# RohanVKashyap/resolution-pde

Measured on AMD Instinct MI355X. Metric: training samples/sec, FFNO2D NS 256^2, higher is better.
Workload: dtype f32; 1 GPU; FFNO2D(1,1,width=64,n_layers=4,n_modes=20,factor=4,ff_weight_norm,n_ff_layers=3,layer_norm,dropout=0.1) train step on [B,1,256,256] Gaussian random fields (BASELINE configs[2]); batch_per_gpu=32, global_batch=32, optimizer=AdamW lr=1e-3 (rpde.optim.FlatAdamW: torch.optim.AdamW's rule, one kernel), parallelism=single, grad_bucket_bytes=6828576, target=input advanced by a fixed spectral filter (utils/synthetic.py:advance)

## Files before the change

resolution-pde_amd/csrc/wgrad_h2.hip:

```cpp
#include "h2.h"
#include "pointwise.h"
#include "wgrad_h2.h"

namespace rpde {

constexpr int WG_WAVES = 8;
constexpr int WG_PANEL = 8192;
constexpr int WG_BLOCKS = 256;

struct WgP {
  const float* a;
  const float* b;
  float* slabs;
  long npts;
  long steps;
  int M, N, nchunk;
  const float* w;
  float* gx;
  int early;
};

template <int PA, int PB, int WM, int WN, int TM, int TN, bool ACT, bool DG = false>
__global__ __launch_bounds__(64 * WG_WAVES, 2) void k_wgrad_h2(const WgP P) {
  static_assert(!DG || (PB == 1 && PA * 2 <= 8), "data gradient: N = 64, M <= 256");
  constexpr int WFRAG = DG ? PA * 2 * 4 * 2048 : 0;
  static_assert(WM * WN == WG_WAVES && PA + PB <= WG_WAVES, "eight waves, one panel per loader wave");
  static_assert(WM * TM * 16 == PA * 64 && WN * TN * 16 == PB * 64, "wave tiles cover the block");
  static_assert((TM * 16) % 64 == 0 || 64 % (TM * 16) == 0, "a wave tile stays inside one panel or covers whole panels");
  constexpr int STAGE = (PA + PB) * WG_PANEL;
  __shared__ __attribute__((aligned(16))) char smem[2 * STAGE + WFRAG];
  __shared__ int einfo[2][WG_WAVES];
  __shared__ float wmax[WG_WAVES];
  const int tid = threadIdx.x, l = tid & 63, wave = tid >> 6, g = l >> 4, li = l & 15;
  const int chunk = blockIdx.x, mblock = blockIdx.y;
  const long s0 = P.steps * chunk / P.nchunk, s1 = P.steps * (chunk + 1) / P.nchunk;

  const bool loader = wave < PA + PB, isA = wave < PA;
  const int ld = isA ? P.M : P.N;
  const float* __restrict__ src = isA ? P.a + mblock * (64 * PA) + 64 * wave : P.b + 64 * (wave - PA);
  src += (long)g * ld + 4 * li;
  float4 buf[8];
  int e_run = 15;
  auto issue = [&](long s) {
    if (!loader || s >= s1) return;
    const float* __restrict__ q0 = src + s * 32 * ld;
    if ((s + 1) * 32 <= P.npts) {
#pragma unroll
      for (int i = 0; i < 8; ++i) buf[i] = *reinterpret_cast<const float4*>(q0 + (long)(4 * i) * ld);
    } else {
#pragma unroll
      for (int i = 0; i < 8; ++i)
        buf[i] = s * 32 + 4 * i + g < P.npts ? *reinterpret_cast<const float4*>(q0 + (long)(4 * i) * ld) : make_float4(0.f, 0.f, 0.f, 0.f);
    }
  };
  auto convert = [&](int st) {
    if (!loader) return;
    if (ACT && !isA) {
#pragma unroll
      for (int i = 0; i < 8; ++i) { buf[i].x = gelu_f(buf[i].x); buf[i].y = gelu_f(buf[i].y); buf[i].z = gelu_f(buf[i].z); buf[i].w = gelu_f(buf[i].w); }
    }
    float m = 0.f;
#pragma unroll
    for (int i = 0; i < 8; ++i) m = fmaxf(fmaxf(m, fmaxf(fabsf(buf[i].x), fabsf(buf[i].y))), fmaxf(fabsf(buf[i].z), fabsf(buf[i].w)));
    m = wave_max(m);
    e_run = max(e_run, (int)(__float_as_uint(m) >> 23) & 0xff);
    e_run = min(e_run, 254);
    const float scale = __uint_as_float((unsigned)(268 - e_run) << 23);
    char* const dst = smem + st * STAGE + wave * WG_PANEL;
#pragma unroll
    for (int i = 0; i < 8; ++i) {
      uint2 hi, lo;
      h2_split4(buf[i].x * scale, buf[i].y * scale, buf[i].z * scale, buf[i].w * scale, hi, lo);
      const int off = stage_off(4 * i + g, li);
      *reinterpret_cast<uint2*>(dst + off) = hi;
      *reinterpret_cast<uint2*>(dst + 4096 + off) = lo;
    }
    if (l == 0) einfo[st][wave] = e_run;
  };

  const int wm = wave / WN, wn = wave % WN;
  const int m_off = wm * TM * 16, n_off = wn * TN * 16;
  const int pa = m_off >> 6, ta0 = (m_off & 63) >> 4, pb = PA + (n_off >> 6), tb0 = (n_off & 63) >> 4;
  const int q = li >> 2, pp = li & 3;
  const int tsw = ((q >> 1) & 1) | ((g & 1) << 1);
  const int trow = (8 * g + q) * 128 + pp * 8;
  typedef s16x4v __attribute__((address_space(3))) * lds_tr;
  auto frag = [&](const char* panel, int tile, f16x8& hi, f16x8& lo) {
    const char* t = panel + trow + ((tile ^ tsw) << 5);
    union { struct { s16x4v a, b; } h; f16x8 v; } uh, ul;
    uh.h.a = __builtin_amdgcn_ds_read_tr16_b64_v4i16((lds_tr)(t));
    uh.h.b = __builtin_amdgcn_ds_read_tr16_b64_v4i16((lds_tr)(t + 512));
    ul.h.a = __builtin_amdgcn_ds_read_tr16_b64_v4i16((lds_tr)(t + 4096));
    ul.h.b = __builtin_amdgcn_ds_read_tr16_b64_v4i16((lds_tr)(t + 4096 + 512));
    hi = uh.v; lo = ul.v;
  };
  f32x4v acc[TM][TN];
#pragma unroll
  for (int i = 0; i < TM; ++i)
#pragma unroll
    for (int j = 0; j < TN; ++j) acc[i][j] = (f32x4v){0.f, 0.f, 0.f, 0.f};
  constexpr int NPA = (TM * 16 + 63) / 64;
  static_assert(TN * 16 <= 64, "one B panel per wave tile");
  int ea_used[NPA], eb_used = 15;
#pragma unroll
  for (int k = 0; k < NPA; ++k) ea_used[k] = 15;

  char* const wfrag = smem + 2 * STAGE;
  float w_inv = 1.f;
  if (DG && s0 < s1) {
    constexpr int NF = PA * 2 * 4 * 64 / (64 * WG_WAVES);
    float wv[NF][8];
    float m = 0.f;
#pragma unroll
    for (int r = 0; r < NF; ++r) {
      const int c = tid + r * 64 * WG_WAVES, fl = c & 63, nt = (c >> 6) & 3, ks = c >> 8;
#pragma unroll
      for (int j = 0; j < 8; ++j) {
        wv[r][j] = P.w[(long)(32 * ks + 8 * (fl >> 4) + j) * P.N + 16 * nt + (fl & 15)];
        m = fmaxf(m, fabsf(wv[r][j]));
      }
    }
    m = wave_max(m);
    if (l == 0) wmax[wave] = m;
    __syncthreads();
    m = 0.f;
#pragma unroll
    for (int i = 0; i < WG_WAVES; ++i) m = fmaxf(m, wmax[i]);
    float w_scale;
    h2_scale(m, 0, w_scale, w_inv);
#pragma unroll
    for (int r = 0; r < NF; ++r) {
      const int c = tid + r * 64 * WG_WAVES, fl = c & 63, nt = (c >> 6) & 3, ks = c >> 8;
      uint2 h0, l0, h1, l1;
      h2_split4(wv[r][0] * w_scale, wv[r][1] * w_scale, wv[r][2] * w_scale, wv[r][3] * w_scale, h0, l0);
      h2_split4(wv[r][4] * w_scale, wv[r][5] * w_scale, wv[r][6] * w_scale, wv[r][7] * w_scale, h1, l1);
      char* d = wfrag + (ks * 4 + nt) * 2048 + fl * 16;
      *reinterpret_cast<uint4*>(d) = make_uint4(h0.x, h0.y, h1.x, h1.y);
      *reinterpret_cast<uint4*>(d + 1024) = make_uint4(l0.x, l0.y, l1.x, l1.y);
    }
  }
  const int dg_mt = wave & 1, dg_nt = wave >> 1;

  const bool early_convert = (P.early >> __builtin_amdgcn_readfirstlane(wave)) & 1;
  if (s0 < s1) {
    issue(s0);
    convert(0);
    issue(s0 + 1);
    lds_barrier();
    for (long s = s0; s < s1; ++s) {
      const int cur = (int)(s - s0) & 1;
      const char* const stage = smem + cur * STAGE;
      if (early_convert && s + 1 < s1) {
        convert(cur ^ 1);
        issue(s + 2);
      }
      const int eb = __builtin_amdgcn_readfirstlane(einfo[cur][pb]);
#pragma unroll
      for (int k = 0; k < NPA; ++k) {
        const int ea = __builtin_amdgcn_readfirstlane(einfo[cur][pa + k]);
        if (ea + eb != ea_used[k] + eb_used) {
          const int d = (ea_used[k] + eb_used) - (ea + eb);
          const float f = d > -126 ? __uint_as_float((unsigned)(127 + d) << 23) : 0.f;
#pragma unroll
          for (int i = 0; i < TM; ++i)
            if (((ta0 + i) >> 2) == k) {
#pragma unroll
              for (int j = 0; j < TN; ++j) acc[i][j] *= f;
            }
        }
        ea_used[k] = ea;
      }
      eb_used = eb;
      f16x8 bh[TN], bl[TN];
#pragma unroll
      for (int j = 0; j < TN; ++j) frag(stage + (pb + ((tb0 + j) >> 2)) * WG_PANEL, (tb0 + j) & 3, bh[j], bl[j]);
#pragma unroll
      for (int i = 0; i < TM; ++i) {
        f16x8 ah, al;
        frag(stage + (pa + ((ta0 + i) >> 2)) * WG_PANEL, (ta0 + i) & 3, ah, al);
#pragma unroll
        for (int j = 0; j < TN; ++j) acc[i][j] = h2_mfma32(ah, al, bh[j], bl[j], acc[i][j]);
      }
      if (DG) {
        f32x4v tot = (f32x4v){0.f, 0.f, 0.f, 0.f};
        const int row = 16 * dg_mt + li;
#pragma unroll
        for (int k = 0; k < PA; ++k) {
          f32x4v part = (f32x4v){0.f, 0.f, 0.f, 0.f};
#pragma unroll
          for (int h = 0; h < 2; ++h) {
            const char* pa_ = stage + k * WG_PANEL + stage_off(row, 2 * (4 * h + g));
            const f16x8 ah = *reinterpret_cast<const f16x8*>(pa_), al = *reinterpret_cast<const f16x8*>(pa_ + 4096);
            const char* wb = wfrag + ((2 * k + h) * 4 + dg_nt) * 2048 + l * 16;
            const f16x8 bh = *reinterpret_cast<const f16x8*>(wb), bl = *reinterpret_cast<const f16x8*>(wb + 1024);
            part = h2_mfma32(ah, al, bh, bl, part);
          }
          const int ek = __builtin_amdgcn_readfirstlane(einfo[cur][k]);
          const float fk = __uint_as_float((unsigned)(ek - 14) << 23) * w_inv;
          tot += part * fk;
        }
        float t0 = tot[0], t1 = tot[1], t2 = tot[2], t3 = tot[3];
        quad_transpose(t0, t1, t2, t3);
        const long pq = s * 32 + 16 * dg_mt + 4 * g + (li & 3);
        if (pq < P.npts) *reinterpret_cast<float4*>(P.gx + pq * P.N + 16 * dg_nt + 4 * (li >> 2)) = make_float4(t0, t1, t2, t3);
      }
      if (!early_convert && s + 1 < s1) {
        convert(cur ^ 1);
        issue(s + 2);
      }
      lds_barrier();
    }
  }

  const float fb = __uint_as_float((unsigned)(eb_used - 14) << 23);
  float* __restrict__ out = P.slabs + (long)chunk * P.M * P.N + (long)(mblock * (64 * PA) + m_off) * P.N + n_off;
#pragma unroll
  for (int i = 0; i < TM; ++i) {
    const float fa = __uint_as_float((unsigned)(ea_used[(ta0 + i) >> 2] - 14) << 23);
#pragma unroll
    for (int j = 0; j < TN; ++j)
#pragma unroll
      for (int r = 0; r < 4; ++r) out[(long)(16 * i + 4 * g + r) * P.N + 16 * j + li] = acc[i][j][r] * fa * fb;
  }
}

bool wgrad_h2_ok(long P, int out_f, int in_f) {
  if (switch_off("RPDE_WGRAD_H2") || P < 32L * WG_BLOCKS) return false;
  return (out_f == 256 && in_f == 256) || (out_f == 256 && in_f == 64) || (out_f == 64 && in_f == 256);
}

static int wg_chunks(int, int) { return WG_BLOCKS; }

static int wg_early_mask(int out_f, int in_f) {
  return out_f == 256 && in_f == 256 ? 0xF0 : (out_f == 64 ? 0x0E : 0x00);
}

size_t wgrad_h2_slab_floats(long P, int out_f, int in_f) {
  return wgrad_h2_ok(P, out_f, in_f) ? (size_t)wg_chunks(out_f, in_f) * out_f * in_f : 0;
}

template <int PA, int PB, int WM, int WN, int TM, int TN>
static void wg_launch(const WgP& p, int mblocks, bool act, hipStream_t st) {
  const dim3 grid(p.nchunk, mblocks);
  if (act) hipLaunchKernelGGL((k_wgrad_h2<PA, PB, WM, WN, TM, TN, true>), grid, dim3(64 * WG_WAVES), 0, st, p);
  else hipLaunchKernelGGL((k_wgrad_h2<PA, PB, WM, WN, TM, TN, false>), grid, dim3(64 * WG_WAVES), 0, st, p);
}

bool wgrad_h2_dgrad_ok(long P, int out_f, int in_f) { return wgrad_h2_ok(P, out_f, in_f) && out_f == 256 && in_f == 64; }

int wgrad_h2_dgrad(const float* gy, const float* h, const float* w, float* gw, float* gx, long P, int in_f, int out_f,
                   float* slabs, hipStream_t st, FoldJobs* defer) {
  RPDE_CHECK_ARG(wgrad_h2_dgrad_ok(P, out_f, in_f) && slabs && w && gx, "wgrad_h2_dgrad: unsupported shape");
  WgP p;
  p.a = gy; p.b = h; p.slabs = slabs; p.npts = P; p.steps = (P + 31) / 32; p.M = out_f; p.N = in_f; p.nchunk = WG_BLOCKS;
  p.early = wg_early_mask(out_f, in_f);
  p.w = w; p.gx = gx;
  hipLaunchKernelGGL((k_wgrad_h2<4, 1, 4, 2, 4, 2, false, true>), dim3(p.nchunk, 1), dim3(64 * WG_WAVES), 0, st, p);
  RPDE_LAUNCH_CHECK();
  if (defer && defer->add(slabs, gw, out_f * in_f, p.nchunk, (long)out_f * in_f)) return RPDE_OK;
  return reduce_slabs(slabs, gw, (long)out_f * in_f, p.nchunk, (long)out_f * in_f, 1.f, 0, st);
}

int wgrad_h2(const float* gy, const float* h, float* gw, long P, int in_f, int out_f, int act_b, float* slabs, hipStream_t st,
             FoldJobs* defer) {
  RPDE_CHECK_ARG(wgrad_h2_ok(P, out_f, in_f) && slabs, "wgrad_h2: unsupported shape");
  RPDE_CHECK_ARG(act_b == RPDE_ACT_IDENTITY || act_b == RPDE_ACT_GELU, "wgrad_h2: activation %d", act_b);
  WgP p;
  p.a = gy; p.b = h; p.slabs = slabs; p.npts = P; p.steps = (P + 31) / 32; p.M = out_f; p.N = in_f; p.nchunk = wg_chunks(out_f, in_f);
  p.early = wg_early_mask(out_f, in_f);
  p.w = nullptr; p.gx = nullptr;
  const bool act = act_b == RPDE_ACT_GELU;
  if (out_f == 256 && in_f == 256) wg_launch<4, 4, 2, 4, 8, 4>(p, 1, act, st);
  else if (out_f == 256) wg_launch<4, 1, 4, 2, 4, 2>(p, 1, act, st);
  else wg_launch<1, 4, 1, 8, 4, 2>(p, 1, act, st);
  RPDE_LAUNCH_CHECK();
  if (defer && defer->add(slabs, gw, out_f * in_f, p.nchunk, (long)out_f * in_f)) return RPDE_OK;
  return reduce_slabs(slabs, gw, (long)out_f * in_f, p.nchunk, (long)out_f * in_f, 1.f, 0, st);
}

}
```

Measured before the change: 1012 samples/s.

## Hold weight fragments in registers and stage data-gradient rows through LDS

In the fused weight-gradient plus data-gradient kernel, the W fragments now stay in registers instead of being read from LDS on every step. Each step's gx tile is written to a double-buffered, XOR-swizzled LDS buffer, and the non-loader waves flush it to global memory one step later as full contiguous rows. The early-convert wave mask for this path also changes. The aim is to cut LDS traffic and scattered global stores on the critical path, at the cost of extra registers per wave. A timestamp profiling mode is added but compiled only under RPDE_STAMPS.

After: 1018 samples/s (median of 6 runs). Within noise of the previous version (+0.6%).

```diff
diff --git a/profiles/wg_stamps.py b/profiles/wg_stamps.py
--- /dev/null
+++ b/profiles/wg_stamps.py
@@ -0,0 +1,31 @@
+#!/usr/bin/env python3
+import ctypes as C
+import os
+import sys
+
+REPO = os.path.dirname(os.path.dirname(os.path.abspath(__file__)))
+for p in (REPO, os.path.join(REPO, "resolution-pde_amd")):
+    sys.path.insert(0, p)
+import numpy as np
+import torch
+from rpde import _lib
+from models.custom_layer import FeedForward
+
+lib = _lib.load()
+ff = FeedForward(64, 4, n_layers=3, layer_norm=True, dropout=0.1).to("cuda")
+x = torch.randn(32, 256, 256, 64, device="cuda").requires_grad_(True)
+res = torch.randn(32, 256, 256, 64, device="cuda")
+g = torch.randn(32, 256, 256, 64, device="cuda")
+for _ in range(3):
+    ff(x, residual=res).backward(g)
+torch.cuda.synchronize()
+buf = (C.c_ulonglong * 64)()
+lib.rpde_debug_wg_stamps.argtypes = [C.c_void_p]
+_lib.check(lib.rpde_debug_wg_stamps(buf), "stamps")
+t = np.array(buf, dtype=np.uint64).reshape(8, 8).astype(np.int64)
+names = ["early convert", "main product", "data gradient", "load wait", "convert", "issue + gx rows", "barrier"]
+print("cycles per step (s_memtime ticks), workgroup 128, steps", int(t[0, 7]))
+print("wave " + " ".join(f"{n:>15s}" for n in names) + "          total")
+for w in range(8):
+    per = t[w, :7] / max(1, t[w, 7])
+    print(f"{w:4d} " + " ".join(f"{v:15.0f}" for v in per) + f" {per.sum():14.0f}")
diff --git a/resolution-pde_amd/csrc/wgrad_h2.hip b/resolution-pde_amd/csrc/wgrad_h2.hip
--- a/resolution-pde_amd/csrc/wgrad_h2.hip
+++ b/resolution-pde_amd/csrc/wgrad_h2.hip
@@ -7,6 +7,14 @@
 constexpr int WG_WAVES = 8;
 constexpr int WG_PANEL = 8192;
 constexpr int WG_BLOCKS = 256;
+
+#ifdef RPDE_STAMPS
+constexpr int WG_NSTAMP = 8;
+__device__ unsigned long long g_wgstamps[WG_WAVES * WG_NSTAMP];
+#define WGSTAMP(i) do { if (DG) { const unsigned long long t_ = __builtin_amdgcn_s_memtime(); st_acc[i] += t_ - st_last; st_last = t_; } } while (0)
+#else
+#define WGSTAMP(i) do {} while (0)
+#endif
 
 struct WgP {
   const float* a;
@@ -23,12 +31,12 @@
 template <int PA, int PB, int WM, int WN, int TM, int TN, bool ACT, bool DG = false>
 __global__ __launch_bounds__(64 * WG_WAVES, 2) void k_wgrad_h2(const WgP P) {
   static_assert(!DG || (PB == 1 && PA * 2 <= 8), "data gradient: N = 64, M <= 256");
-  constexpr int WFRAG = DG ? PA * 2 * 4 * 2048 : 0;
   static_assert(WM * WN == WG_WAVES && PA + PB <= WG_WAVES, "eight waves, one panel per loader wave");
   static_assert(WM * TM * 16 == PA * 64 && WN * TN * 16 == PB * 64, "wave tiles cover the block");
   static_assert((TM * 16) % 64 == 0 || 64 % (TM * 16) == 0, "a wave tile stays inside one panel or covers whole panels");
   constexpr int STAGE = (PA + PB) * WG_PANEL;
-  __shared__ __attribute__((aligned(16))) char smem[2 * STAGE + WFRAG];
+  constexpr int GXBUF = 32 * 64 * 4;
+  __shared__ __attribute__((aligned(16))) char smem[2 * STAGE + (DG ? 2 * GXBUF : 0)];
   __shared__ int einfo[2][WG_WAVES];
   __shared__ float wmax[WG_WAVES];
   const int tid = threadIdx.x, l = tid & 63, wave = tid >> 6, g = l >> 4, li = l & 15;
@@ -105,21 +113,20 @@
 #pragma unroll
   for (int k = 0; k < NPA; ++k) ea_used[k] = 15;
 
-  char* const wfrag = smem + 2 * STAGE;
+  const int dg_mt = wave & 1, dg_nt = wave >> 1;
+  constexpr int NKS = DG ? PA * 2 : 1;
+  f16x8 wh[NKS], wl[NKS];
   float w_inv = 1.f;
   if (DG && s0 < s1) {
-    constexpr int NF = PA * 2 * 4 * 64 / (64 * WG_WAVES);
-    float wv[NF][8];
+    float wv[NKS][8];
     float m = 0.f;
 #pragma unroll
-    for (int r = 0; r < NF; ++r) {
-      const int c = tid + r * 64 * WG_WAVES, fl = c & 63, nt = (c >> 6) & 3, ks = c >> 8;
+    for (int ks = 0; ks < NKS; ++ks)
 #pragma unroll
       for (int j = 0; j < 8; ++j) {
-        wv[r][j] = P.w[(long)(32 * ks + 8 * (fl >> 4) + j) * P.N + 16 * nt + (fl & 15)];
-        m = fmaxf(m, fabsf(wv[r][j]));
-      }
-    }
+        wv[ks][j] = P.w[(long)(32 * ks + 8 * g + j) * P.N + 16 * dg_nt + li];
+        m = fmaxf(m, fabsf(wv[ks][j]));
+      }
     m = wave_max(m);
     if (l == 0) wmax[wave] = m;
     __syncthreads();
@@ -129,17 +136,29 @@
     float w_scale;
     h2_scale(m, 0, w_scale, w_inv);
 #pragma unroll
-    for (int r = 0; r < NF; ++r) {
-      const int c = tid + r * 64 * WG_WAVES, fl = c & 63, nt = (c >> 6) & 3, ks = c >> 8;
-      uint2 h0, l0, h1, l1;
-      h2_split4(wv[r][0] * w_scale, wv[r][1] * w_scale, wv[r][2] * w_scale, wv[r][3] * w_scale, h0, l0);
-      h2_split4(wv[r][4] * w_scale, wv[r][5] * w_scale, wv[r][6] * w_scale, wv[r][7] * w_scale, h1, l1);
-      char* d = wfrag + (ks * 4 + nt) * 2048 + fl * 16;
-      *reinterpret_cast<uint4*>(d) = make_uint4(h0.x, h0.y, h1.x, h1.y);
-      *reinterpret_cast<uint4*>(d + 1024) = make_uint4(l0.x, l0.y, l1.x, l1.y);
+    for (int ks = 0; ks < NKS; ++ks) {
+#pragma unroll
+      for (int j = 0; j < 8; ++j) wv[ks][j] *= w_scale;
+      h2_frag(wv[ks], wh[ks], wl[ks]);
     }
   }
-  const int dg_mt = wave & 1, dg_nt = wave >> 1;
+
+  char* const gxs = smem + 2 * STAGE;
+  auto gx_flush = [&](long sp, int b) {
+    constexpr int W0 = PA + PB, NW = WG_WAVES - W0;
+    static_assert(!DG || NW > 0, "data gradient: at least one wave without a panel");
+    if (!DG || wave < W0) return;
+#pragma unroll
+    for (int rg = 0; rg < 8; rg += NW) {
+      const int r = rg + wave - W0;
+      if (r < 8) {
+        const int prow = 4 * r + g;
+        const float4 v = *reinterpret_cast<const float4*>(gxs + b * GXBUF + prow * 256 + ((li ^ ((prow & 3) << 2)) << 4));
+        const long pq = sp * 32 + prow;
+        if (pq < P.npts) *reinterpret_cast<float4*>(P.gx + pq * P.N + 4 * li) = v;
+      }
+    }
+  };
 
   const bool early_convert = (P.early >> __builtin_amdgcn_readfirstlane(wave)) & 1;
   if (s0 < s1) {
@@ -147,6 +166,9 @@
     convert(0);
     issue(s0 + 1);
     lds_barrier();
+#ifdef RPDE_STAMPS
+    unsigned long long st_acc[WG_NSTAMP] = {0, 0, 0, 0, 0, 0, 0, 0}, st_last = __builtin_amdgcn_s_memtime();
+#endif
     for (long s = s0; s < s1; ++s) {
       const int cur = (int)(s - s0) & 1;
       const char* const stage = smem + cur * STAGE;
@@ -154,6 +176,7 @@
         convert(cur ^ 1);
         issue(s + 2);
       }
+      WGSTAMP(0);
       const int eb = __builtin_amdgcn_readfirstlane(einfo[cur][pb]);
 #pragma unroll
       for (int k = 0; k < NPA; ++k) {
@@ -181,6 +204,7 @@
 #pragma unroll
         for (int j = 0; j < TN; ++j) acc[i][j] = h2_mfma32(ah, al, bh[j], bl[j], acc[i][j]);
       }
+      WGSTAMP(1);
       if (DG) {
         f32x4v tot = (f32x4v){0.f, 0.f, 0.f, 0.f};
         const int row = 16 * dg_mt + li;
@@ -191,9 +215,7 @@
           for (int h = 0; h < 2; ++h) {
             const char* pa_ = stage + k * WG_PANEL + stage_off(row, 2 * (4 * h + g));
             const f16x8 ah = *reinterpret_cast<const f16x8*>(pa_), al = *reinterpret_cast<const f16x8*>(pa_ + 4096);
-            const char* wb = wfrag + ((2 * k + h) * 4 + dg_nt) * 2048 + l * 16;
-            const f16x8 bh = *reinterpret_cast<const f16x8*>(wb), bl = *reinterpret_cast<const f16x8*>(wb + 1024);
-            part = h2_mfma32(ah, al, bh, bl, part);
+            part = h2_mfma32(ah, al, wh[2 * k + h], wl[2 * k + h], part);
           }
           const int ek = __builtin_amdgcn_readfirstlane(einfo[cur][k]);
           const float fk = __uint_as_float((unsigned)(ek - 14) << 23) * w_inv;
@@ -201,15 +223,32 @@
         }
         float t0 = tot[0], t1 = tot[1], t2 = tot[2], t3 = tot[3];
         quad_transpose(t0, t1, t2, t3);
-        const long pq = s * 32 + 16 * dg_mt + 4 * g + (li & 3);
-        if (pq < P.npts) *reinterpret_cast<float4*>(P.gx + pq * P.N + 16 * dg_nt + 4 * (li >> 2)) = make_float4(t0, t1, t2, t3);
-      }
+        const int prow = 16 * dg_mt + 4 * g + (li & 3), c = 4 * dg_nt + (li >> 2);
+        *reinterpret_cast<float4*>(gxs + cur * GXBUF + prow * 256 + ((c ^ ((prow & 3) << 2)) << 4)) = make_float4(t0, t1, t2, t3);
+      }
+      WGSTAMP(2);
+#ifdef RPDE_STAMPS
+      if (DG) asm volatile("s_waitcnt vmcnt(0)" ::: "memory");
+      WGSTAMP(3);
+#endif
       if (!early_convert && s + 1 < s1) {
         convert(cur ^ 1);
+        WGSTAMP(4);
         issue(s + 2);
       }
+      if (DG && s > s0) gx_flush(s - 1, cur ^ 1);
+      WGSTAMP(5);
       lds_barrier();
-    }
+      WGSTAMP(6);
+    }
+#ifdef RPDE_STAMPS
+    if (DG && blockIdx.x == WG_BLOCKS / 2 && l == 0) {
+#pragma unroll
+      for (int i = 0; i < WG_NSTAMP - 1; ++i) g_wgstamps[wave * WG_NSTAMP + i] = st_acc[i];
+      g_wgstamps[wave * WG_NSTAMP + WG_NSTAMP - 1] = (unsigned long long)(s1 - s0);
+    }
+#endif
+    if (DG) gx_flush(s1 - 1, (int)(s1 - 1 - s0) & 1);
   }
 
   const float fb = __uint_as_float((unsigned)(eb_used - 14) << 23);
@@ -234,6 +273,7 @@
 static int wg_early_mask(int out_f, int in_f) {
   return out_f == 256 && in_f == 256 ? 0xF0 : (out_f == 64 ? 0x0E : 0x00);
 }
+constexpr int WG_EARLY_DG = 0x1C;
 
 size_t wgrad_h2_slab_floats(long P, int out_f, int in_f) {
   return wgrad_h2_ok(P, out_f, in_f) ? (size_t)wg_chunks(out_f, in_f) * out_f * in_f : 0;
@@ -253,7 +293,7 @@
   RPDE_CHECK_ARG(wgrad_h2_dgrad_ok(P, out_f, in_f) && slabs && w && gx, "wgrad_h2_dgrad: unsupported shape");
   WgP p;
   p.a = gy; p.b = h; p.slabs = slabs; p.npts = P; p.steps = (P + 31) / 32; p.M = out_f; p.N = in_f; p.nchunk = WG_BLOCKS;
-  p.early = wg_early_mask(out_f, in_f);
+  p.early = WG_EARLY_DG;
   p.w = w; p.gx = gx;
   hipLaunchKernelGGL((k_wgrad_h2<4, 1, 4, 2, 4, 2, false, true>), dim3(p.nchunk, 1), dim3(64 * WG_WAVES), 0, st, p);
   RPDE_LAUNCH_CHECK();
@@ -279,3 +319,11 @@
 }
 
 }
+
+#ifdef RPDE_STAMPS
+extern "C" int rpde_debug_wg_stamps(unsigned long long* host_out) {
+  RPDE_HIP(hipDeviceSynchronize());
+  RPDE_HIP(hipMemcpyFromSymbol(host_out, HIP_SYMBOL(rpde::g_wgstamps), sizeof(unsigned long long) * rpde::WG_WAVES * rpde::WG_NSTAMP));
+  return RPDE_OK;
+}
+#endif
```
